# duylebkHCM/EyeDiseaseSegmentation

Hardware: NVIDIA B200
Metric: IDRiD-size (2848x4288) fundus images/s, 4 lesion models, sliding-window + 8-view D4 TTA + AUC-PR (higher is better)
Workload: dtype bf16

## Files before the change

eyediseasesegmentation_b200/csrc/conv3x3_wide_sm100.cu:

```cuda
#include "tc_ptx.cuh"
#include <algorithm>
#include <cstring>
#include <mutex>

namespace eds {

constexpr int kWideThreads = 320;
constexpr int kWideStagesMax = 4;
constexpr int kWideRows = 8, kWideSlabCols = 32, kWideOutCols = 30, kWideSlabRows = kWideRows + 2;

struct WideParams {
    CUtensorMap a_map;
    CUtensorMap a_map1;
    int k_split;
    CUtensorMap b_map;
    CUtensorMap y_map;
    const float* bias;
    const __nv_bfloat16* residual;
    __nv_bfloat16* y;
    int C, block_k, k_chunks, bn;
    int N, H, W, relu;
    int tiles_w, tiles_h, total_tiles;
    int stages, atom_bytes, a_slab_bytes, b_box_bytes, stage_bytes, tmem_cols;
    int b_resident, b_region_bytes;
    int staged, staging_off;
    uint32_t idesc, desc_hi;
};

__device__ __forceinline__ void wide_mbar_arrive(uint64_t* bar) {
    asm volatile("mbarrier.arrive.shared::cta.b64 _, [%0];" ::"r"(smem_u32(bar)) : "memory");
}

__global__ void __launch_bounds__(kWideThreads, 1)
conv3x3_wide_kernel(const __grid_constant__ WideParams p) {
    extern __shared__ uint8_t smem_raw[];
    uint8_t* smem = reinterpret_cast<uint8_t*>((reinterpret_cast<uintptr_t>(smem_raw) + 1023) & ~(uintptr_t)1023);
    uint8_t* ring = smem + p.b_region_bytes;
    uint64_t* full_bar = reinterpret_cast<uint64_t*>(ring + (size_t)p.stages * p.stage_bytes);
    uint64_t* empty_bar = full_bar + kWideStagesMax;
    uint64_t* tmem_full_bar = empty_bar + kWideStagesMax;
    uint64_t* tmem_empty_bar = tmem_full_bar + 2;
    uint64_t* b_bar = tmem_empty_bar + 2;
    uint32_t* tmem_slot = reinterpret_cast<uint32_t*>(b_bar + 1);
    float* s_bias = reinterpret_cast<float*>(full_bar + 16);
    if (threadIdx.x < (unsigned)p.bn) s_bias[threadIdx.x] = p.bias ? __ldg(p.bias + threadIdx.x) : 0.f;

    const int warp = threadIdx.x >> 5, lane = threadIdx.x & 31;
    if (warp == 0 && lane == 0) {
        prefetch_tmap(&p.a_map);
        prefetch_tmap(&p.a_map1);
        prefetch_tmap(&p.b_map);
        for (int s = 0; s < p.stages; ++s) {
            mbar_init(&full_bar[s], 1);
            mbar_init(&empty_bar[s], 1);
        }
        for (int m = 0; m < 2; ++m) {
            mbar_init(&tmem_full_bar[m], 1);
            mbar_init(&tmem_empty_bar[m], 4);
        }
        mbar_init(b_bar, 1);
        asm volatile("fence.mbarrier_init.release.cluster;" ::: "memory");
        asm volatile("fence.proxy.async.shared::cta;" ::: "memory");
    }
    if (warp == 1) tmem_alloc(tmem_slot, (uint32_t)p.tmem_cols);
    tc_fence_before();
    __syncthreads();
    tc_fence_after();
    const uint32_t tmem_base = *tmem_slot;
    const uint32_t n3 = 3u * (uint32_t)p.bn;

    if (warp == 0) {
        if (lane == 0) {
            int stage = 0;
            uint32_t phase = 0;
            const uint32_t a_tx = (uint32_t)(kWideSlabRows * 4 * p.atom_bytes), b_tx = (uint32_t)(9 * p.bn * p.block_k * 2);
            const uint32_t tx = p.b_resident ? a_tx : a_tx + b_tx;
            if (p.b_resident) {
                mbar_arrive_expect_tx(b_bar, b_tx * (uint32_t)p.k_chunks);
                for (int kc = 0; kc < p.k_chunks; ++kc)
                    for (int tap = 0; tap < 9; ++tap)
                        tma_load_2d(smem + (size_t)(kc * 9 + tap) * p.b_box_bytes, &p.b_map, b_bar,
                                    tap * p.C + kc * p.block_k, 0);
            }
            for (int tile = blockIdx.x; tile < p.total_tiles; tile += gridDim.x) {
                const int tw = tile % p.tiles_w;
                const int t2 = tile / p.tiles_w;
                const int th = t2 % p.tiles_h;
                const int n = t2 / p.tiles_h;
                const int w0 = tw * kWideOutCols, h0 = th * kWideRows;
                for (int kc = 0; kc < p.k_chunks; ++kc) {
                    mbar_wait(&empty_bar[stage], phase ^ 1u);
                    mbar_arrive_expect_tx(&full_bar[stage], tx);
                    uint8_t* sa = ring + (size_t)stage * p.stage_bytes;
                    uint8_t* sb = sa + p.a_slab_bytes;
                    if (kc < p.k_split)
                        tma_load_4d(sa, &p.a_map, &full_bar[stage], kc * p.block_k, w0 - 1, h0 - 1, n);
                    else
                        tma_load_4d(sa, &p.a_map1, &full_bar[stage], (kc - p.k_split) * p.block_k, w0 - 1, h0 - 1, n);
                    if (!p.b_resident)
                        for (int tap = 0; tap < 9; ++tap)
                            tma_load_2d(sb + tap * p.b_box_bytes, &p.b_map, &full_bar[stage], tap * p.C + kc * p.block_k, 0);
                    if (++stage == p.stages) { stage = 0; phase ^= 1u; }
                }
            }
        }
    } else if (warp == 1) {
        int stage = 0;
        uint32_t phase = 0;
        const uint32_t lo0 = desc_lo(smem_u32(ring)), blo0 = desc_lo(smem_u32(smem));
        const uint32_t stage16 = (uint32_t)p.stage_bytes >> 4, slab16 = (uint32_t)p.a_slab_bytes >> 4;
        const uint32_t bchunk16 = 9u * ((uint32_t)p.b_box_bytes >> 4);
        if (p.b_resident) mbar_wait(b_bar, 0);
        const uint32_t atom16 = (uint32_t)p.atom_bytes >> 4, brow16 = 3u * ((uint32_t)p.b_box_bytes >> 4);
        const uint32_t dhi_w = p.desc_hi, idesc = p.idesc;
        const int k_steps = p.block_k / 16;
        int t = 0;
        for (int tile = blockIdx.x; tile < p.total_tiles; tile += gridDim.x, ++t) {
            const uint32_t empty_parity = (uint32_t)((t & 1) ^ 1);
            for (int kc = 0; kc < p.k_chunks; ++kc) {
                mbar_wait(&full_bar[stage], phase);
                const uint32_t a_st = lo0 + (uint32_t)stage * stage16;
                const uint32_t b_st = p.b_resident ? blo0 + (uint32_t)kc * bchunk16 : a_st + slab16;
#pragma unroll
                for (int m = 0; m < 2; ++m) {
                    if (kc == 0) mbar_wait(&tmem_empty_bar[m], empty_parity);
                    tc_fence_after();
                    if (elect_one()) {
                        const uint32_t d = tmem_base + (uint32_t)m * n3;
#pragma unroll
                        for (int dhi = 0; dhi < 3; ++dhi) {
                            const uint32_t a_lo = a_st + (uint32_t)(m * 16 + dhi * 4) * atom16;
                            const uint32_t b_lo = b_st + (uint32_t)dhi * brow16;
                            for (int ks = 0; ks < k_steps; ++ks)
                                umma_bf16_lohi(d, a_lo + 2u * ks, b_lo + 2u * ks, dhi_w, idesc,
                                               (kc > 0 || dhi > 0 || ks > 0) ? 1u : 0u);
                        }
                    }
                    __syncwarp();
                    if (kc == p.k_chunks - 1) {
                        if (elect_one()) umma_commit(&tmem_full_bar[m]);
                        __syncwarp();
                    }
                }
                if (elect_one()) umma_commit(&empty_bar[stage]);
                __syncwarp();
                if (++stage == p.stages) { stage = 0; phase ^= 1u; }
            }
        }
    } else {
        const int q = warp & 3;
        const int m = (warp - 2) >> 2;
        const int bn = p.bn;
        uint8_t* stg = smem + p.staging_off + (size_t)(warp - 2) * 4096;
        const int pos = lane - 1;
        int t = 0;
        for (int tile = blockIdx.x; tile < p.total_tiles; tile += gridDim.x, ++t) {
            const int tw = tile % p.tiles_w;
            const int t2 = tile / p.tiles_w;
            const int th = t2 % p.tiles_h;
            const int n = t2 / p.tiles_h;
            const int ow = tw * kWideOutCols - 1 + lane;
            const bool col_ok = lane >= 1 && lane <= kWideOutCols && ow < p.W;
            {
                mbar_wait(&tmem_full_bar[m], (uint32_t)(t & 1));
                tc_fence_after();
                const int oh = th * kWideRows + m * 4 + q;
                const bool valid = col_ok && oh < p.H;
                const int64_t off = (((int64_t)n * p.H + oh) * p.W + ow) * bn;
                const uint32_t taddr = tmem_base + ((uint32_t)(q * 32) << 16) + (uint32_t)m * n3;
                if (p.staged) {
                    if (lane == 0) asm volatile("cp.async.bulk.wait_group.read 0;" ::: "memory");
                    __syncwarp();
                }
                for (int c = 0; c < bn; c += 16) {
                    uint32_t rl[16], rc[16], rr[16];
                    tmem_ld16_nowait(taddr + (uint32_t)c, rl);
                    tmem_ld16_nowait(taddr + (uint32_t)(bn + c), rc);
                    tmem_ld16_nowait(taddr + (uint32_t)(2 * bn + c), rr);
                    tmem_ld_wait();
                    float v[16];
#pragma unroll
                    for (int i = 0; i < 16; ++i) {
                        const float l = __shfl_up_sync(0xffffffffu, __uint_as_float(rl[i]), 1);
                        const float r = __shfl_down_sync(0xffffffffu, __uint_as_float(rr[i]), 1);
                        v[i] = (l + __uint_as_float(rc[i])) + r;
                    }
                    if (valid || (p.staged && pos >= 0 && pos < kWideOutCols)) {
                        {
                            const float4* b4 = reinterpret_cast<const float4*>(s_bias + c);
#pragma unroll
                            for (int i = 0; i < 4; ++i) {
                                const float4 b = b4[i];
                                v[4 * i] += b.x; v[4 * i + 1] += b.y; v[4 * i + 2] += b.z; v[4 * i + 3] += b.w;
                            }
                        }
                        if (p.residual && valid) {
                            float r0[8], r1[8];
                            Vec8<__nv_bfloat16>::ld(p.residual + off + c, r0);
                            Vec8<__nv_bfloat16>::ld(p.residual + off + c + 8, r1);
#pragma unroll
                            for (int i = 0; i < 8; ++i) { v[i] += r0[i]; v[8 + i] += r1[i]; }
                        }
                        if (p.relu) {
#pragma unroll
                            for (int i = 0; i < 16; ++i) v[i] = fmaxf(v[i], 0.f);
                        }
                        float o0[8], o1[8];
#pragma unroll
                        for (int i = 0; i < 8; ++i) { o0[i] = v[i]; o1[i] = v[8 + i]; }
                        if (p.staged) {
                            const uint32_t j = (uint32_t)c >> 3, sw = (uint32_t)pos & 7u;
                            Vec8<__nv_bfloat16>::st(reinterpret_cast<__nv_bfloat16*>(stg + pos * 128 + ((j ^ sw) << 4)), o0);
                            Vec8<__nv_bfloat16>::st(reinterpret_cast<__nv_bfloat16*>(stg + pos * 128 + (((j + 1) ^ sw) << 4)), o1);
                        } else {
                            Vec8<__nv_bfloat16>::st(p.y + off + c, o0);
                            Vec8<__nv_bfloat16>::st(p.y + off + c + 8, o1);
                        }
                    }
                }
                if (p.staged) {
                    asm volatile("fence.proxy.async.shared::cta;" ::: "memory");
                    __syncwarp();
                    if (lane == 0 && oh < p.H) {
                        asm volatile(
                            "cp.async.bulk.tensor.4d.global.shared::cta.bulk_group [%0, {%2, %3, %4, %5}], [%1];"
                            ::"l"(&p.y_map), "r"(smem_u32(stg)), "r"(0), "r"(tw * kWideOutCols), "r"(oh), "r"(n)
                            : "memory");
                        asm volatile("cp.async.bulk.commit_group;" ::: "memory");
                    }
                }
                tc_fence_before();
                __syncwarp();
                if (lane == 0) wide_mbar_arrive(&tmem_empty_bar[m]);
            }
        }
        if (p.staged && lane == 0) asm volatile("cp.async.bulk.wait_group 0;" ::: "memory");
    }

    tc_fence_before();
    __syncthreads();
    if (warp == 1) tmem_dealloc(tmem_base, (uint32_t)p.tmem_cols);
}

static PerDevice g_wide_once;
static int g_wide_sms = 148;

static int wide_init() {
    return g_wide_once.run([](int dev) {
        cudaError_t e = cudaFuncSetAttribute(conv3x3_wide_kernel, cudaFuncAttributeMaxDynamicSharedMemorySize, 227 * 1024);
        if (e != cudaSuccess) {
            set_error("conv3x3_wide: cannot opt in to 227 KB shared memory: %s", cudaGetErrorString(e));
            return (int)EDS_ERR_CUDA;
        }
        int sms = 0;
        if (cudaDeviceGetAttribute(&sms, cudaDevAttrMultiProcessorCount, dev) == cudaSuccess && sms > 0) g_wide_sms = sms;
        return (int)EDS_OK;
    });
}

}

using namespace eds;

extern "C" int eds_conv3x3_wide_supported(int C, int Cout, int R, int S, int stride, int pad) {
    return R == 3 && S == 3 && stride == 1 && pad == 1 && C >= 16 && C % 16 == 0 && Cout >= 16 && Cout % 16 == 0 &&
           Cout <= 64;
}

static int wide_launch(const void* x, int C0, const void* x1, int C1, int N, int H, int W, const void* w,
                       const float* bias, int Cout, int relu, const void* residual, void* y, void* stream) {
    const int C = C0 + C1;
    EDS_REQUIRE(x && w && y, "conv3x3_wide: null pointer");
    EDS_REQUIRE(C0 >= 16 && C0 % 16 == 0 && C1 >= 0 && C1 % 16 == 0 && (x1 != nullptr) == (C1 > 0),
                "conv3x3_wide: C0=%d C1=%d must be multiples of 16", C0, C1);
    EDS_REQUIRE(N > 0 && H > 0 && W > 0, "conv3x3_wide: bad shape N=%d H=%d W=%d", N, H, W);
    EDS_REQUIRE(eds_conv3x3_wide_supported(C, Cout, 3, 3, 1, 1),
                "conv3x3_wide: C=%d Cout=%d outside the supported range (multiples of 16, Cout <= 64)", C, Cout);
    EDS_REQUIRE((((uintptr_t)x | (uintptr_t)x1 | (uintptr_t)w | (uintptr_t)y | (uintptr_t)residual | (uintptr_t)bias) &
                 15) == 0, "conv3x3_wide: pointers must be 16-byte aligned");
    if (int rc = igemm_init()) return rc;
    if (int rc = wide_init()) return rc;

    WideParams p;
    memset(&p, 0, sizeof(p));
    p.bias = bias;
    p.residual = (const __nv_bfloat16*)residual;
    p.y = (__nv_bfloat16*)y;
    p.C = C;
    p.block_k = ((C0 | C1) % 64 == 0) ? 64 : ((C0 | C1) % 32 == 0 ? 32 : 16);
    p.k_chunks = C / p.block_k;
    p.k_split = C0 / p.block_k;
    p.bn = Cout;
    p.N = N; p.H = H; p.W = W; p.relu = relu;
    p.tiles_w = ceil_div(W, kWideOutCols);
    p.tiles_h = ceil_div(H, kWideRows);
    const int64_t total = (int64_t)p.tiles_w * p.tiles_h * N;
    EDS_REQUIRE(total < (1ll << 31), "conv3x3_wide: too many tiles");
    p.total_tiles = (int)total;

    const CUtensorMapSwizzle swz = p.block_k == 64 ? CU_TENSOR_MAP_SWIZZLE_128B
                                  : p.block_k == 32 ? CU_TENSOR_MAP_SWIZZLE_64B : CU_TENSOR_MAP_SWIZZLE_32B;
    const uint32_t layout = p.block_k == 64 ? 2u : (p.block_k == 32 ? 4u : 6u);
    p.atom_bytes = 8 * p.block_k * 2;
    const uint32_t sbo = (uint32_t)p.atom_bytes >> 4;
    p.desc_hi = sbo | (1u << 14) | (layout << 29);
    p.idesc = (1u << 4) | (1u << 7) | (1u << 10) | ((uint32_t)((3 * p.bn) >> 3) << 17) | ((uint32_t)(128 >> 4) << 24);
    p.a_slab_bytes = (kWideSlabRows * 4 * p.atom_bytes + 1023) & ~1023;
    p.b_box_bytes = p.bn * p.block_k * 2;
    const int barrier_bytes = 128 + 64 * 4;
    const int budget = 227 * 1024 - 1024 - barrier_bytes;
    const int b_all = p.k_chunks * 9 * p.b_box_bytes;
    p.b_resident = b_all + 3 * p.a_slab_bytes <= budget;
    p.b_region_bytes = p.b_resident ? ((b_all + 1023) & ~1023) : 0;
    p.stage_bytes = p.b_resident ? p.a_slab_bytes : ((p.a_slab_bytes + 9 * p.b_box_bytes + 1023) & ~1023);
    p.stages = std::min(kWideStagesMax, (budget - p.b_region_bytes) / p.stage_bytes);
    EDS_REQUIRE(p.stages >= 2, "conv3x3_wide: a stage of %d B leaves no room for double buffering", p.stage_bytes);
    int cols = 32;
    while (cols < 6 * p.bn) cols <<= 1;
    p.tmem_cols = cols;
    const int after_bars = p.b_region_bytes + p.stages * p.stage_bytes + barrier_bytes;
    p.staging_off = (after_bars + 1023) & ~1023;
    p.staged = p.bn == 64 && p.block_k == 64 && p.staging_off + 8 * 4096 + 1024 <= 227 * 1024;
    const size_t smem = (p.staged ? (size_t)p.staging_off + 8 * 4096 : (size_t)after_bars) + 1024;
    EDS_REQUIRE(smem <= 227 * 1024 && p.tmem_cols <= 512, "conv3x3_wide: tile does not fit (smem %zu, tmem %d)", smem,
                p.tmem_cols);

    {
        cuuint64_t dims[4] = {(cuuint64_t)C0, (cuuint64_t)W, (cuuint64_t)H, (cuuint64_t)N};
        cuuint64_t strides[3] = {(cuuint64_t)C0 * 2, (cuuint64_t)W * C0 * 2, (cuuint64_t)H * W * C0 * 2};
        cuuint32_t box[4] = {(cuuint32_t)p.block_k, (cuuint32_t)kWideSlabCols, (cuuint32_t)kWideSlabRows, 1u};
        if (int rc = tmap_encode_bf16(&p.a_map, x, 4, dims, strides, box, swz, "wide input")) return rc;
        p.a_map1 = p.a_map;
    }
    if (x1) {
        cuuint64_t dims[4] = {(cuuint64_t)C1, (cuuint64_t)W, (cuuint64_t)H, (cuuint64_t)N};
        cuuint64_t strides[3] = {(cuuint64_t)C1 * 2, (cuuint64_t)W * C1 * 2, (cuuint64_t)H * W * C1 * 2};
        cuuint32_t box[4] = {(cuuint32_t)p.block_k, (cuuint32_t)kWideSlabCols, (cuuint32_t)kWideSlabRows, 1u};
        if (int rc = tmap_encode_bf16(&p.a_map1, x1, 4, dims, strides, box, swz, "wide second input")) return rc;
    }
    {
        cuuint64_t dims[2] = {(cuuint64_t)9 * C, (cuuint64_t)Cout};
        cuuint64_t strides[1] = {(cuuint64_t)9 * C * 2};
        cuuint32_t box[2] = {(cuuint32_t)p.block_k, (cuuint32_t)p.bn};
        if (int rc = tmap_encode_bf16(&p.b_map, w, 2, dims, strides, box, swz, "wide weights")) return rc;
    }
    if (p.staged) {
        cuuint64_t dims[4] = {(cuuint64_t)Cout, (cuuint64_t)W, (cuuint64_t)H, (cuuint64_t)N};
        cuuint64_t strides[3] = {(cuuint64_t)Cout * 2, (cuuint64_t)W * Cout * 2, (cuuint64_t)H * W * Cout * 2};
        cuuint32_t box[4] = {64u, (cuuint32_t)kWideOutCols, 1u, 1u};
        if (int rc = tmap_encode_bf16(&p.y_map, y, 4, dims, strides, box, CU_TENSOR_MAP_SWIZZLE_128B, "wide output")) return rc;
    }
    const int grid = (int)std::min<int64_t>(total, g_wide_sms);
    conv3x3_wide_kernel<<<grid, kWideThreads, smem, as_stream(stream)>>>(p);
    return check_launch("conv3x3_wide_kernel");
}

extern "C" int eds_conv3x3_wide_bf16(const void* x, int N, int H, int W, int C, const void* w, const float* bias,
                                     int Cout, int relu, const void* residual, void* y, void* stream) {
    return wide_launch(x, C, nullptr, 0, N, H, W, w, bias, Cout, relu, residual, y, stream);
}

extern "C" int eds_conv3x3_wide_bf16_2src(const void* x0, int C0, const void* x1, int C1, int N, int H, int W,
                                          const void* w, const float* bias, int Cout, int relu, const void* residual,
                                          void* y, void* stream) {
    EDS_REQUIRE(x1 && C1 > 0, "conv3x3_wide_2src: second input missing");
    return wide_launch(x0, C0, x1, C1, N, H, W, w, bias, Cout, relu, residual, y, stream);
}
```

eyediseasesegmentation_b200/csrc/tc_ptx.cuh:

```cuda
#pragma once
#include "common.cuh"
#include <cuda.h>

namespace eds {

__device__ __forceinline__ uint32_t smem_u32(const void* p) { return (uint32_t)__cvta_generic_to_shared(p); }

__device__ __forceinline__ void mbar_init(uint64_t* bar, uint32_t count) {
    asm volatile("mbarrier.init.shared::cta.b64 [%0], %1;" ::"r"(smem_u32(bar)), "r"(count) : "memory");
}
__device__ __forceinline__ void mbar_arrive_expect_tx(uint64_t* bar, uint32_t bytes) {
    asm volatile("mbarrier.arrive.expect_tx.shared::cta.b64 _, [%0], %1;" ::"r"(smem_u32(bar)), "r"(bytes)
                 : "memory");
}
__device__ __forceinline__ bool mbar_try_wait(uint64_t* bar, uint32_t parity) {
    uint32_t ok;
    asm volatile(
        "{\n\t.reg .pred p;\n\t"
        "mbarrier.try_wait.parity.shared::cta.b64 p, [%1], %2;\n\t"
        "selp.u32 %0, 1, 0, p;\n\t}"
        : "=r"(ok)
        : "r"(smem_u32(bar)), "r"(parity)
        : "memory");
    return ok != 0;
}
__device__ __forceinline__ void mbar_wait(uint64_t* bar, uint32_t parity) {
    if (mbar_try_wait(bar, parity)) return;
    const long long t0 = clock64();
    while (!mbar_try_wait(bar, parity)) {
        if (clock64() - t0 > 4000000000LL) {
            printf("eds conv_igemm: mbarrier timeout (block %d thread %d)\n", (int)blockIdx.x, (int)threadIdx.x);
            __trap();
        }
    }
}
__device__ __forceinline__ void tma_load_4d(void* dst, const CUtensorMap* map, uint64_t* bar, int c0, int c1, int c2,
                                            int c3) {
    asm volatile(
        "cp.async.bulk.tensor.4d.shared::cluster.global.mbarrier::complete_tx::bytes [%0], [%1, {%3, %4, %5, %6}], [%2];"
        ::"r"(smem_u32(dst)), "l"(map), "r"(smem_u32(bar)), "r"(c0), "r"(c1), "r"(c2), "r"(c3)
        : "memory");
}
__device__ __forceinline__ void tma_load_2d(void* dst, const CUtensorMap* map, uint64_t* bar, int c0, int c1) {
    asm volatile(
        "cp.async.bulk.tensor.2d.shared::cluster.global.mbarrier::complete_tx::bytes [%0], [%1, {%3, %4}], [%2];"
        ::"r"(smem_u32(dst)), "l"(map), "r"(smem_u32(bar)), "r"(c0), "r"(c1)
        : "memory");
}
__device__ __forceinline__ void prefetch_tmap(const CUtensorMap* map) {
    asm volatile("prefetch.tensormap [%0];" ::"l"(map) : "memory");
}
__device__ __forceinline__ void tc_fence_before() { asm volatile("tcgen05.fence::before_thread_sync;" ::: "memory"); }
__device__ __forceinline__ void tc_fence_after() { asm volatile("tcgen05.fence::after_thread_sync;" ::: "memory"); }
__device__ __forceinline__ void tmem_alloc(uint32_t* dst, uint32_t cols) {
    asm volatile("tcgen05.alloc.cta_group::1.sync.aligned.shared::cta.b32 [%0], %1;" ::"r"(smem_u32(dst)), "r"(cols)
                 : "memory");
    asm volatile("tcgen05.relinquish_alloc_permit.cta_group::1.sync.aligned;" ::: "memory");
}
__device__ __forceinline__ void tmem_dealloc(uint32_t addr, uint32_t cols) {
    asm volatile("tcgen05.dealloc.cta_group::1.sync.aligned.b32 %0, %1;" ::"r"(addr), "r"(cols) : "memory");
}
__device__ __forceinline__ void umma_bf16(uint32_t tmem_d, uint64_t desc_a, uint64_t desc_b, uint32_t idesc,
                                          uint32_t accumulate) {
    asm volatile(
        "{\n\t.reg .pred p;\n\t"
        "setp.ne.b32 p, %4, 0;\n\t"
        "tcgen05.mma.cta_group::1.kind::f16 [%0], %1, %2, %3, p;\n\t}"
        ::"r"(tmem_d), "l"(desc_a), "l"(desc_b), "r"(idesc), "r"(accumulate)
        : "memory");
}
__device__ __forceinline__ void umma_commit(uint64_t* bar) {
    asm volatile("tcgen05.commit.cta_group::1.mbarrier::arrive::one.shared::cluster.b64 [%0];" ::"r"(smem_u32(bar))
                 : "memory");
}
__device__ __forceinline__ void tmem_ld16(uint32_t taddr, uint32_t (&r)[16]) {
    asm volatile(
        "tcgen05.ld.sync.aligned.32x32b.x16.b32 "
        "{%0, %1, %2, %3, %4, %5, %6, %7, %8, %9, %10, %11, %12, %13, %14, %15}, [%16];"
        : "=r"(r[0]), "=r"(r[1]), "=r"(r[2]), "=r"(r[3]), "=r"(r[4]), "=r"(r[5]), "=r"(r[6]), "=r"(r[7]), "=r"(r[8]),
          "=r"(r[9]), "=r"(r[10]), "=r"(r[11]), "=r"(r[12]), "=r"(r[13]), "=r"(r[14]), "=r"(r[15])
        : "r"(taddr)
        : "memory");
    asm volatile("tcgen05.wait::ld.sync.aligned;" ::: "memory");
}

__device__ __forceinline__ void tmem_ld16_nowait(uint32_t taddr, uint32_t (&r)[16]) {
    asm volatile(
        "tcgen05.ld.sync.aligned.32x32b.x16.b32 "
        "{%0, %1, %2, %3, %4, %5, %6, %7, %8, %9, %10, %11, %12, %13, %14, %15}, [%16];"
        : "=r"(r[0]), "=r"(r[1]), "=r"(r[2]), "=r"(r[3]), "=r"(r[4]), "=r"(r[5]), "=r"(r[6]), "=r"(r[7]), "=r"(r[8]),
          "=r"(r[9]), "=r"(r[10]), "=r"(r[11]), "=r"(r[12]), "=r"(r[13]), "=r"(r[14]), "=r"(r[15])
        : "r"(taddr)
        : "memory");
}
__device__ __forceinline__ void tmem_ld_wait() { asm volatile("tcgen05.wait::ld.sync.aligned;" ::: "memory"); }

__device__ __forceinline__ bool elect_one() {
    uint32_t pred;
    asm volatile(
        "{\n\t.reg .pred p;\n\t"
        "elect.sync _|p, 0xffffffff;\n\t"
        "selp.u32 %0, 1, 0, p;\n\t}"
        : "=r"(pred));
    return pred != 0;
}
__device__ __forceinline__ void umma_bf16_lohi(uint32_t tmem_d, uint32_t a_lo, uint32_t b_lo, uint32_t desc_hi,
                                               uint32_t idesc, uint32_t accumulate) {
    asm volatile(
        "{\n\t.reg .pred p;\n\t.reg .b64 da, db;\n\t"
        "setp.ne.b32 p, %5, 0;\n\t"
        "mov.b64 da, {%1, %3};\n\t"
        "mov.b64 db, {%2, %3};\n\t"
        "tcgen05.mma.cta_group::1.kind::f16 [%0], da, db, %4, p;\n\t}"
        ::"r"(tmem_d), "r"(a_lo), "r"(b_lo), "r"(desc_hi), "r"(idesc), "r"(accumulate)
        : "memory");
}
__device__ __forceinline__ uint32_t desc_lo(uint32_t saddr) { return ((saddr & 0x3FFFFu) >> 4) | (1u << 16); }

__device__ __forceinline__ uint64_t make_desc(uint32_t saddr, uint32_t desc_hi) {
    return (uint64_t)(((saddr & 0x3FFFFu) >> 4) | (1u << 16)) | ((uint64_t)desc_hi << 32);
}


int tmap_encode_bf16(CUtensorMap* map, const void* base, int rank, const cuuint64_t* dims, const cuuint64_t* strides,
                     const cuuint32_t* box, CUtensorMapSwizzle swz, const char* what);
int igemm_init();

}
```

Before: 1.890.

## Run wide 3x3 conv as 2-CTA cluster pairs with split weight loads

Adds a cta_group::2 variant of the wide implicit-GEMM 3x3 convolution. Two CTAs in a cluster each load their own activation slab and half of the weight boxes, and the leader issues M=256 paired UMMAs, with commits multicast to both CTAs and cross-CTA TMEM-empty arrivals. This halves per-CTA weight shared-memory traffic and footprint, allowing more pipeline stages (max raised to 5). It adds cluster synchronisation, a drain loop and an occupancy query, and risks load imbalance from odd tile counts and extra handshake latency.

```diff
diff --git a/eyediseasesegmentation_b200/csrc/conv3x3_wide_sm100.cu b/eyediseasesegmentation_b200/csrc/conv3x3_wide_sm100.cu
--- a/eyediseasesegmentation_b200/csrc/conv3x3_wide_sm100.cu
+++ b/eyediseasesegmentation_b200/csrc/conv3x3_wide_sm100.cu
@@ -2,11 +2,13 @@
 #include <algorithm>
 #include <cstring>
 #include <mutex>
+#include <utility>
+#include <vector>
 
 namespace eds {
 
 constexpr int kWideThreads = 320;
-constexpr int kWideStagesMax = 4;
+constexpr int kWideStagesMax = 5;
 constexpr int kWideRows = 8, kWideSlabCols = 32, kWideOutCols = 30, kWideSlabRows = kWideRows + 2;
 
 struct WideParams {
@@ -20,17 +22,30 @@
     __nv_bfloat16* y;
     int C, block_k, k_chunks, bn;
     int N, H, W, relu;
-    int tiles_w, tiles_h, total_tiles;
+    int tiles_w, tiles_h, total_tiles, total_pairs;
     int stages, atom_bytes, a_slab_bytes, b_box_bytes, stage_bytes, tmem_cols;
     int b_resident, b_region_bytes;
     int staged, staging_off;
     uint32_t idesc, desc_hi;
 };
 
-__device__ __forceinline__ void wide_mbar_arrive(uint64_t* bar) {
-    asm volatile("mbarrier.arrive.shared::cta.b64 _, [%0];" ::"r"(smem_u32(bar)) : "memory");
-}
-
+template <int kCtas> __device__ __forceinline__ void wide_commit(uint64_t* bar) {
+    if constexpr (kCtas == 2) umma_commit_pair(bar);
+    else umma_commit(bar);
+}
+template <int kCtas>
+__device__ __forceinline__ void wide_tma_4d(void* dst, const CUtensorMap* map, uint64_t* bar, int c0, int c1, int c2,
+                                            int c3) {
+    if constexpr (kCtas == 2) tma_load_4d_pair(dst, map, cluster_addr(bar, 0), c0, c1, c2, c3);
+    else tma_load_4d(dst, map, bar, c0, c1, c2, c3);
+}
+template <int kCtas>
+__device__ __forceinline__ void wide_tma_2d(void* dst, const CUtensorMap* map, uint64_t* bar, int c0, int c1) {
+    if constexpr (kCtas == 2) tma_load_2d_pair(dst, map, cluster_addr(bar, 0), c0, c1);
+    else tma_load_2d(dst, map, bar, c0, c1);
+}
+
+template <int kCtas>
 __global__ void __launch_bounds__(kWideThreads, 1)
 conv3x3_wide_kernel(const __grid_constant__ WideParams p) {
     extern __shared__ uint8_t smem_raw[];
@@ -46,6 +61,8 @@
     if (threadIdx.x < (unsigned)p.bn) s_bias[threadIdx.x] = p.bias ? __ldg(p.bias + threadIdx.x) : 0.f;
 
     const int warp = threadIdx.x >> 5, lane = threadIdx.x & 31;
+    const uint32_t rank = kCtas == 2 ? cluster_ctarank() : 0u;
+    const int pair0 = (int)blockIdx.x / kCtas, pair_step = (int)gridDim.x / kCtas;
     if (warp == 0 && lane == 0) {
         prefetch_tmap(&p.a_map);
         prefetch_tmap(&p.a_map1);
@@ -56,15 +73,19 @@
         }
         for (int m = 0; m < 2; ++m) {
             mbar_init(&tmem_full_bar[m], 1);
-            mbar_init(&tmem_empty_bar[m], 4);
+            mbar_init(&tmem_empty_bar[m], 4 * kCtas);
         }
         mbar_init(b_bar, 1);
         asm volatile("fence.mbarrier_init.release.cluster;" ::: "memory");
         asm volatile("fence.proxy.async.shared::cta;" ::: "memory");
     }
-    if (warp == 1) tmem_alloc(tmem_slot, (uint32_t)p.tmem_cols);
+    if (warp == 1) {
+        if constexpr (kCtas == 2) tmem_alloc_pair(tmem_slot, (uint32_t)p.tmem_cols);
+        else tmem_alloc(tmem_slot, (uint32_t)p.tmem_cols);
+    }
     tc_fence_before();
-    __syncthreads();
+    if constexpr (kCtas == 2) cluster_sync();
+    else __syncthreads();
     tc_fence_after();
     const uint32_t tmem_base = *tmem_slot;
     const uint32_t n3 = 3u * (uint32_t)p.bn;
@@ -73,16 +94,23 @@
         if (lane == 0) {
             int stage = 0;
             uint32_t phase = 0;
-            const uint32_t a_tx = (uint32_t)(kWideSlabRows * 4 * p.atom_bytes), b_tx = (uint32_t)(9 * p.bn * p.block_k * 2);
-            const uint32_t tx = p.b_resident ? a_tx : a_tx + b_tx;
+            const int hb = p.bn >> 1, nb = 6 / kCtas;
+            const uint32_t a_tx = (uint32_t)(kWideSlabRows * 4 * p.atom_bytes), b_tx = (uint32_t)(3 * nb * p.b_box_bytes);
+            const uint32_t tx = (uint32_t)kCtas * (p.b_resident ? a_tx : a_tx + b_tx);
+            auto load_b = [&](uint8_t* sb, uint64_t* bar, int kc) {
+                for (int dh = 0; dh < 3; ++dh)
+                    for (int i = 0; i < nb; ++i) {
+                        const int j = nb * (int)rank + i;
+                        wide_tma_2d<kCtas>(sb + (dh * nb + i) * p.b_box_bytes, &p.b_map, bar,
+                                           (dh * 3 + (j >> 1)) * p.C + kc * p.block_k, (j & 1) * hb);
+                    }
+            };
             if (p.b_resident) {
-                mbar_arrive_expect_tx(b_bar, b_tx * (uint32_t)p.k_chunks);
-                for (int kc = 0; kc < p.k_chunks; ++kc)
-                    for (int tap = 0; tap < 9; ++tap)
-                        tma_load_2d(smem + (size_t)(kc * 9 + tap) * p.b_box_bytes, &p.b_map, b_bar,
-                                    tap * p.C + kc * p.block_k, 0);
+                if (rank == 0) mbar_arrive_expect_tx(b_bar, (uint32_t)kCtas * b_tx * (uint32_t)p.k_chunks);
+                for (int kc = 0; kc < p.k_chunks; ++kc) load_b(smem + (size_t)kc * b_tx, b_bar, kc);
             }
-            for (int tile = blockIdx.x; tile < p.total_tiles; tile += gridDim.x) {
+            for (int pt = pair0; pt < p.total_pairs; pt += pair_step) {
+                const int tile = kCtas * pt + (int)rank;
                 const int tw = tile % p.tiles_w;
                 const int t2 = tile / p.tiles_w;
                 const int th = t2 % p.tiles_h;
@@ -90,77 +118,92 @@
                 const int w0 = tw * kWideOutCols, h0 = th * kWideRows;
                 for (int kc = 0; kc < p.k_chunks; ++kc) {
                     mbar_wait(&empty_bar[stage], phase ^ 1u);
-                    mbar_arrive_expect_tx(&full_bar[stage], tx);
+                    if (rank == 0) mbar_arrive_expect_tx(&full_bar[stage], tx);
+                    uint64_t* bar = &full_bar[stage];
                     uint8_t* sa = ring + (size_t)stage * p.stage_bytes;
                     uint8_t* sb = sa + p.a_slab_bytes;
                     if (kc < p.k_split)
-                        tma_load_4d(sa, &p.a_map, &full_bar[stage], kc * p.block_k, w0 - 1, h0 - 1, n);
+                        wide_tma_4d<kCtas>(sa, &p.a_map, bar, kc * p.block_k, w0 - 1, h0 - 1, n);
                     else
-                        tma_load_4d(sa, &p.a_map1, &full_bar[stage], (kc - p.k_split) * p.block_k, w0 - 1, h0 - 1, n);
-                    if (!p.b_resident)
-                        for (int tap = 0; tap < 9; ++tap)
-                            tma_load_2d(sb + tap * p.b_box_bytes, &p.b_map, &full_bar[stage], tap * p.C + kc * p.block_k, 0);
+                        wide_tma_4d<kCtas>(sa, &p.a_map1, bar, (kc - p.k_split) * p.block_k, w0 - 1, h0 - 1, n);
+                    if (!p.b_resident) load_b(sb, bar, kc);
                     if (++stage == p.stages) { stage = 0; phase ^= 1u; }
                 }
             }
+            for (int s = 0; s < p.stages; ++s) {
+                mbar_wait(&empty_bar[stage], phase ^ 1u);
+                if (++stage == p.stages) { stage = 0; phase ^= 1u; }
+            }
         }
     } else if (warp == 1) {
-        int stage = 0;
-        uint32_t phase = 0;
-        const uint32_t lo0 = desc_lo(smem_u32(ring)), blo0 = desc_lo(smem_u32(smem));
-        const uint32_t stage16 = (uint32_t)p.stage_bytes >> 4, slab16 = (uint32_t)p.a_slab_bytes >> 4;
-        const uint32_t bchunk16 = 9u * ((uint32_t)p.b_box_bytes >> 4);
-        if (p.b_resident) mbar_wait(b_bar, 0);
-        const uint32_t atom16 = (uint32_t)p.atom_bytes >> 4, brow16 = 3u * ((uint32_t)p.b_box_bytes >> 4);
-        const uint32_t dhi_w = p.desc_hi, idesc = p.idesc;
-        const int k_steps = p.block_k / 16;
-        int t = 0;
-        for (int tile = blockIdx.x; tile < p.total_tiles; tile += gridDim.x, ++t) {
-            const uint32_t empty_parity = (uint32_t)((t & 1) ^ 1);
-            for (int kc = 0; kc < p.k_chunks; ++kc) {
-                mbar_wait(&full_bar[stage], phase);
-                const uint32_t a_st = lo0 + (uint32_t)stage * stage16;
-                const uint32_t b_st = p.b_resident ? blo0 + (uint32_t)kc * bchunk16 : a_st + slab16;
-#pragma unroll
-                for (int m = 0; m < 2; ++m) {
-                    if (kc == 0) mbar_wait(&tmem_empty_bar[m], empty_parity);
-                    tc_fence_after();
-                    if (elect_one()) {
-                        const uint32_t d = tmem_base + (uint32_t)m * n3;
-#pragma unroll
-                        for (int dhi = 0; dhi < 3; ++dhi) {
-                            const uint32_t a_lo = a_st + (uint32_t)(m * 16 + dhi * 4) * atom16;
-                            const uint32_t b_lo = b_st + (uint32_t)dhi * brow16;
-                            for (int ks = 0; ks < k_steps; ++ks)
-                                umma_bf16_lohi(d, a_lo + 2u * ks, b_lo + 2u * ks, dhi_w, idesc,
-                                               (kc > 0 || dhi > 0 || ks > 0) ? 1u : 0u);
+        if (rank == 0) {
+            int stage = 0;
+            uint32_t phase = 0;
+            const uint32_t lo0 = desc_lo(smem_u32(ring)), blo0 = desc_lo(smem_u32(smem));
+            const uint32_t stage16 = (uint32_t)p.stage_bytes >> 4, slab16 = (uint32_t)p.a_slab_bytes >> 4;
+            const uint32_t brow16 = (uint32_t)(6 / kCtas) * ((uint32_t)p.b_box_bytes >> 4), bchunk16 = 3u * brow16;
+            if (p.b_resident) mbar_wait(b_bar, 0);
+            const uint32_t atom16 = (uint32_t)p.atom_bytes >> 4;
+            const uint32_t dhi_w = p.desc_hi, idesc = p.idesc;
+            const int k_steps = p.block_k / 16;
+            int t = 0;
+            for (int pt = pair0; pt < p.total_pairs; pt += pair_step, ++t) {
+                const uint32_t empty_parity = (uint32_t)((t & 1) ^ 1);
+                for (int kc = 0; kc < p.k_chunks; ++kc) {
+                    mbar_wait(&full_bar[stage], phase);
+                    const uint32_t a_st = lo0 + (uint32_t)stage * stage16;
+                    const uint32_t b_st = p.b_resident ? blo0 + (uint32_t)kc * bchunk16 : a_st + slab16;
+#pragma unroll
+                    for (int m = 0; m < 2; ++m) {
+                        if (kc == 0) {
+                            if constexpr (kCtas == 2) mbar_wait_cluster(&tmem_empty_bar[m], empty_parity);
+                            else mbar_wait(&tmem_empty_bar[m], empty_parity);
+                        }
+                        tc_fence_after();
+                        if (elect_one()) {
+                            const uint32_t d = tmem_base + (uint32_t)m * n3;
+#pragma unroll
+                            for (int dhi = 0; dhi < 3; ++dhi) {
+                                const uint32_t a_lo = a_st + (uint32_t)(m * 16 + dhi * 4) * atom16;
+                                const uint32_t b_lo = b_st + (uint32_t)dhi * brow16;
+                                for (int ks = 0; ks < k_steps; ++ks) {
+                                    const uint32_t acc = (kc > 0 || dhi > 0 || ks > 0) ? 1u : 0u;
+                                    if constexpr (kCtas == 2)
+                                        umma_bf16_pair_lohi(d, a_lo + 2u * ks, b_lo + 2u * ks, dhi_w, idesc, acc);
+                                    else
+                                        umma_bf16_lohi(d, a_lo + 2u * ks, b_lo + 2u * ks, dhi_w, idesc, acc);
+                                }
+                            }
+                        }
+                        __syncwarp();
+                        if (kc == p.k_chunks - 1) {
+                            if (elect_one()) wide_commit<kCtas>(&tmem_full_bar[m]);
+                            __syncwarp();
                         }
                     }
+                    if (elect_one()) wide_commit<kCtas>(&empty_bar[stage]);
                     __syncwarp();
-                    if (kc == p.k_chunks - 1) {
-                        if (elect_one()) umma_commit(&tmem_full_bar[m]);
-                        __syncwarp();
-                    }
-                }
-                if (elect_one()) umma_commit(&empty_bar[stage]);
-                __syncwarp();
-                if (++stage == p.stages) { stage = 0; phase ^= 1u; }
+                    if (++stage == p.stages) { stage = 0; phase ^= 1u; }
+                }
             }
         }
     } else {
         const int q = warp & 3;
         const int m = (warp - 2) >> 2;
         const int bn = p.bn;
+        const uint32_t empty_bar_leader = kCtas == 2 ? cluster_addr(&tmem_empty_bar[m], 0) : 0u;
         uint8_t* stg = smem + p.staging_off + (size_t)(warp - 2) * 4096;
         const int pos = lane - 1;
         int t = 0;
-        for (int tile = blockIdx.x; tile < p.total_tiles; tile += gridDim.x, ++t) {
+        for (int pt = pair0; pt < p.total_pairs; pt += pair_step, ++t) {
+            const int tile = kCtas * pt + (int)rank;
+            const bool tile_ok = tile < p.total_tiles;
             const int tw = tile % p.tiles_w;
             const int t2 = tile / p.tiles_w;
             const int th = t2 % p.tiles_h;
             const int n = t2 / p.tiles_h;
             const int ow = tw * kWideOutCols - 1 + lane;
-            const bool col_ok = lane >= 1 && lane <= kWideOutCols && ow < p.W;
+            const bool col_ok = tile_ok && lane >= 1 && lane <= kWideOutCols && ow < p.W;
             {
                 mbar_wait(&tmem_full_bar[m], (uint32_t)(t & 1));
                 tc_fence_after();
@@ -221,7 +264,7 @@
                 if (p.staged) {
                     asm volatile("fence.proxy.async.shared::cta;" ::: "memory");
                     __syncwarp();
-                    if (lane == 0 && oh < p.H) {
+                    if (lane == 0 && tile_ok && oh < p.H) {
                         asm volatile(
                             "cp.async.bulk.tensor.4d.global.shared::cta.bulk_group [%0, {%2, %3, %4, %5}], [%1];"
                             ::"l"(&p.y_map), "r"(smem_u32(stg)), "r"(0), "r"(tw * kWideOutCols), "r"(oh), "r"(n)
@@ -231,29 +274,78 @@
                 }
                 tc_fence_before();
                 __syncwarp();
-                if (lane == 0) wide_mbar_arrive(&tmem_empty_bar[m]);
+                if (lane == 0) {
+                    if constexpr (kCtas == 2) mbar_arrive_cluster(empty_bar_leader);
+                    else asm volatile("mbarrier.arrive.shared::cta.b64 _, [%0];" ::"r"(smem_u32(&tmem_empty_bar[m])) : "memory");
+                }
             }
         }
         if (p.staged && lane == 0) asm volatile("cp.async.bulk.wait_group 0;" ::: "memory");
     }
 
     tc_fence_before();
-    __syncthreads();
-    if (warp == 1) tmem_dealloc(tmem_base, (uint32_t)p.tmem_cols);
+    if constexpr (kCtas == 2) cluster_sync();
+    else __syncthreads();
+    tc_fence_after();
+    if (warp == 1) {
+        if constexpr (kCtas == 2) tmem_dealloc_pair(tmem_base, (uint32_t)p.tmem_cols);
+        else tmem_dealloc(tmem_base, (uint32_t)p.tmem_cols);
+    }
 }
 
 static PerDevice g_wide_once;
-static int g_wide_sms = 148;
+static int g_wide_sms[kMaxDevices];
+
+static cudaLaunchConfig_t wide_pair_config(int grid, size_t smem, cudaStream_t stream, cudaLaunchAttribute* attr) {
+    cudaLaunchConfig_t cfg = {};
+    cfg.gridDim = dim3((unsigned)grid);
+    cfg.blockDim = dim3(kWideThreads);
+    cfg.dynamicSmemBytes = smem;
+    cfg.stream = stream;
+    attr->id = cudaLaunchAttributeClusterDimension;
+    attr->val.clusterDim.x = 2;
+    attr->val.clusterDim.y = 1;
+    attr->val.clusterDim.z = 1;
+    cfg.attrs = attr;
+    cfg.numAttrs = 1;
+    return cfg;
+}
+
+static int wide_max_pairs(size_t smem) {
+    static std::mutex mu;
+    static std::vector<std::pair<std::pair<int, size_t>, int>> cache;
+    int dev = 0;
+    if (cudaGetDevice(&dev) != cudaSuccess) return 0;
+    std::lock_guard<std::mutex> lock(mu);
+    for (const auto& e : cache)
+        if (e.first.first == dev && e.first.second == smem) return e.second;
+    cudaLaunchAttribute attr;
+    const cudaLaunchConfig_t cfg = wide_pair_config(2 * g_wide_sms[dev], smem, nullptr, &attr);
+    int pairs = 0;
+    if (cudaOccupancyMaxActiveClusters(&pairs, conv3x3_wide_kernel<2>, &cfg) != cudaSuccess || pairs <= 0) {
+        (void)cudaGetLastError();
+        return 0;
+    }
+    cache.push_back({{dev, smem}, pairs});
+    return pairs;
+}
 
 static int wide_init() {
     return g_wide_once.run([](int dev) {
-        cudaError_t e = cudaFuncSetAttribute(conv3x3_wide_kernel, cudaFuncAttributeMaxDynamicSharedMemorySize, 227 * 1024);
+        cudaError_t e = cudaFuncSetAttribute(conv3x3_wide_kernel<1>, cudaFuncAttributeMaxDynamicSharedMemorySize, 227 * 1024);
+        if (e == cudaSuccess)
+            e = cudaFuncSetAttribute(conv3x3_wide_kernel<2>, cudaFuncAttributeMaxDynamicSharedMemorySize, 227 * 1024);
         if (e != cudaSuccess) {
             set_error("conv3x3_wide: cannot opt in to 227 KB shared memory: %s", cudaGetErrorString(e));
             return (int)EDS_ERR_CUDA;
         }
         int sms = 0;
-        if (cudaDeviceGetAttribute(&sms, cudaDevAttrMultiProcessorCount, dev) == cudaSuccess && sms > 0) g_wide_sms = sms;
+        e = cudaDeviceGetAttribute(&sms, cudaDevAttrMultiProcessorCount, dev);
+        if (e != cudaSuccess || sms < 2) {
+            set_error("conv3x3_wide: cannot read the SM count: %s", cudaGetErrorString(e));
+            return (int)EDS_ERR_CUDA;
+        }
+        g_wide_sms[dev] = sms;
         return (int)EDS_OK;
     });
 }
@@ -288,8 +380,6 @@
     p.y = (__nv_bfloat16*)y;
     p.C = C;
     p.block_k = ((C0 | C1) % 64 == 0) ? 64 : ((C0 | C1) % 32 == 0 ? 32 : 16);
-    p.k_chunks = C / p.block_k;
-    p.k_split = C0 / p.block_k;
     p.bn = Cout;
     p.N = N; p.H = H; p.W = W; p.relu = relu;
     p.tiles_w = ceil_div(W, kWideOutCols);
@@ -298,29 +388,44 @@
     EDS_REQUIRE(total < (1ll << 31), "conv3x3_wide: too many tiles");
     p.total_tiles = (int)total;
 
+    const int barrier_bytes = 128 + 64 * 4;
+    const int budget = 227 * 1024 - 1024 - barrier_bytes;
+    int ctas = 0;
+    for (;;) {
+        p.k_chunks = C / p.block_k;
+        p.k_split = C0 / p.block_k;
+        p.atom_bytes = 8 * p.block_k * 2;
+        p.a_slab_bytes = (kWideSlabRows * 4 * p.atom_bytes + 1023) & ~1023;
+        p.b_box_bytes = (p.bn / 2) * p.block_k * 2;
+        const int b_whole = p.k_chunks * 18 * p.b_box_bytes;
+        if (ctas == 0) ctas = b_whole + 3 * p.a_slab_bytes <= budget ? 1 : 2;
+        const int b_all = b_whole / ctas;
+        p.b_resident = b_all + 3 * p.a_slab_bytes <= budget;
+        p.b_region_bytes = p.b_resident ? ((b_all + 1023) & ~1023) : 0;
+        p.stage_bytes = p.b_resident ? p.a_slab_bytes : ((p.a_slab_bytes + 18 / ctas * p.b_box_bytes + 1023) & ~1023);
+        const int staging_bytes = 8 * 4096;
+        const int ring_room = budget - p.b_region_bytes;
+        p.staged = p.bn == 64 && ring_room - staging_bytes - 1024 >= 2 * p.stage_bytes;
+        p.stages = std::min(kWideStagesMax, (ring_room - (p.staged ? staging_bytes + 1024 : 0)) / p.stage_bytes);
+        if (ctas == 2 && !p.b_resident && p.block_k == 64 && p.stages < 3) {
+            p.block_k = 32;
+            continue;
+        }
+        break;
+    }
+    EDS_REQUIRE(p.stages >= 2, "conv3x3_wide: a stage of %d B leaves no room for double buffering", p.stage_bytes);
+    p.total_pairs = (int)ceil_div64(total, ctas);
     const CUtensorMapSwizzle swz = p.block_k == 64 ? CU_TENSOR_MAP_SWIZZLE_128B
                                   : p.block_k == 32 ? CU_TENSOR_MAP_SWIZZLE_64B : CU_TENSOR_MAP_SWIZZLE_32B;
     const uint32_t layout = p.block_k == 64 ? 2u : (p.block_k == 32 ? 4u : 6u);
-    p.atom_bytes = 8 * p.block_k * 2;
-    const uint32_t sbo = (uint32_t)p.atom_bytes >> 4;
-    p.desc_hi = sbo | (1u << 14) | (layout << 29);
-    p.idesc = (1u << 4) | (1u << 7) | (1u << 10) | ((uint32_t)((3 * p.bn) >> 3) << 17) | ((uint32_t)(128 >> 4) << 24);
-    p.a_slab_bytes = (kWideSlabRows * 4 * p.atom_bytes + 1023) & ~1023;
-    p.b_box_bytes = p.bn * p.block_k * 2;
-    const int barrier_bytes = 128 + 64 * 4;
-    const int budget = 227 * 1024 - 1024 - barrier_bytes;
-    const int b_all = p.k_chunks * 9 * p.b_box_bytes;
-    p.b_resident = b_all + 3 * p.a_slab_bytes <= budget;
-    p.b_region_bytes = p.b_resident ? ((b_all + 1023) & ~1023) : 0;
-    p.stage_bytes = p.b_resident ? p.a_slab_bytes : ((p.a_slab_bytes + 9 * p.b_box_bytes + 1023) & ~1023);
-    p.stages = std::min(kWideStagesMax, (budget - p.b_region_bytes) / p.stage_bytes);
-    EDS_REQUIRE(p.stages >= 2, "conv3x3_wide: a stage of %d B leaves no room for double buffering", p.stage_bytes);
+    p.desc_hi = ((uint32_t)p.atom_bytes >> 4) | (1u << 14) | (layout << 29);
+    p.idesc = (1u << 4) | (1u << 7) | (1u << 10) | ((uint32_t)((3 * p.bn) >> 3) << 17) |
+              ((uint32_t)(128 * ctas >> 4) << 24);
     int cols = 32;
     while (cols < 6 * p.bn) cols <<= 1;
     p.tmem_cols = cols;
     const int after_bars = p.b_region_bytes + p.stages * p.stage_bytes + barrier_bytes;
     p.staging_off = (after_bars + 1023) & ~1023;
-    p.staged = p.bn == 64 && p.block_k == 64 && p.staging_off + 8 * 4096 + 1024 <= 227 * 1024;
     const size_t smem = (p.staged ? (size_t)p.staging_off + 8 * 4096 : (size_t)after_bars) + 1024;
     EDS_REQUIRE(smem <= 227 * 1024 && p.tmem_cols <= 512, "conv3x3_wide: tile does not fit (smem %zu, tmem %d)", smem,
                 p.tmem_cols);
@@ -341,7 +446,7 @@
     {
         cuuint64_t dims[2] = {(cuuint64_t)9 * C, (cuuint64_t)Cout};
         cuuint64_t strides[1] = {(cuuint64_t)9 * C * 2};
-        cuuint32_t box[2] = {(cuuint32_t)p.block_k, (cuuint32_t)p.bn};
+        cuuint32_t box[2] = {(cuuint32_t)p.block_k, (cuuint32_t)(p.bn / 2)};
         if (int rc = tmap_encode_bf16(&p.b_map, w, 2, dims, strides, box, swz, "wide weights")) return rc;
     }
     if (p.staged) {
@@ -350,8 +455,23 @@
         cuuint32_t box[4] = {64u, (cuuint32_t)kWideOutCols, 1u, 1u};
         if (int rc = tmap_encode_bf16(&p.y_map, y, 4, dims, strides, box, CU_TENSOR_MAP_SWIZZLE_128B, "wide output")) return rc;
     }
-    const int grid = (int)std::min<int64_t>(total, g_wide_sms);
-    conv3x3_wide_kernel<<<grid, kWideThreads, smem, as_stream(stream)>>>(p);
+    int dev = 0;
+    EDS_REQUIRE(cudaGetDevice(&dev) == cudaSuccess, "conv3x3_wide: no current device");
+    if (ctas == 1) {
+        const int grid = std::min(p.total_pairs, g_wide_sms[dev]);
+        conv3x3_wide_kernel<1><<<grid, kWideThreads, smem, as_stream(stream)>>>(p);
+        return check_launch("conv3x3_wide_kernel");
+    }
+    const int max_pairs = wide_max_pairs(smem);
+    EDS_REQUIRE(max_pairs > 0, "conv3x3_wide: a CTA pair with %zu B of shared memory cannot be resident", smem);
+    const int pairs = std::min({p.total_pairs, max_pairs, g_wide_sms[dev] / 2});
+    cudaLaunchAttribute attr;
+    const cudaLaunchConfig_t cfg = wide_pair_config(2 * pairs, smem, as_stream(stream), &attr);
+    const cudaError_t e = cudaLaunchKernelEx(&cfg, conv3x3_wide_kernel<2>, p);
+    if (e != cudaSuccess) {
+        set_error("conv3x3_wide: launch of the CTA-pair kernel failed: %s", cudaGetErrorString(e));
+        return (int)EDS_ERR_CUDA;
+    }
     return check_launch("conv3x3_wide_kernel");
 }
 
diff --git a/eyediseasesegmentation_b200/csrc/tc_ptx.cuh b/eyediseasesegmentation_b200/csrc/tc_ptx.cuh
--- a/eyediseasesegmentation_b200/csrc/tc_ptx.cuh
+++ b/eyediseasesegmentation_b200/csrc/tc_ptx.cuh
@@ -117,6 +117,85 @@
 }
 __device__ __forceinline__ uint32_t desc_lo(uint32_t saddr) { return ((saddr & 0x3FFFFu) >> 4) | (1u << 16); }
 
+__device__ __forceinline__ uint32_t cluster_ctarank() {
+    uint32_t r;
+    asm volatile("mov.u32 %0, %%cluster_ctarank;" : "=r"(r));
+    return r;
+}
+__device__ __forceinline__ void cluster_sync() {
+    asm volatile("barrier.cluster.arrive.release.aligned;\n\tbarrier.cluster.wait.acquire.aligned;" ::: "memory");
+}
+__device__ __forceinline__ uint32_t cluster_addr(const void* p, uint32_t rank) {
+    uint32_t r;
+    asm volatile("mapa.shared::cluster.u32 %0, %1, %2;" : "=r"(r) : "r"(smem_u32(p)), "r"(rank));
+    return r;
+}
+__device__ __forceinline__ bool mbar_try_wait_cluster(uint64_t* bar, uint32_t parity) {
+    uint32_t ok;
+    asm volatile(
+        "{\n\t.reg .pred p;\n\t"
+        "mbarrier.try_wait.parity.acquire.cluster.shared::cta.b64 p, [%1], %2;\n\t"
+        "selp.u32 %0, 1, 0, p;\n\t}"
+        : "=r"(ok)
+        : "r"(smem_u32(bar)), "r"(parity)
+        : "memory");
+    return ok != 0;
+}
+__device__ __forceinline__ void mbar_wait_cluster(uint64_t* bar, uint32_t parity) {
+    if (mbar_try_wait_cluster(bar, parity)) return;
+    const long long t0 = clock64();
+    while (!mbar_try_wait_cluster(bar, parity)) {
+        if (clock64() - t0 > 4000000000LL) {
+            printf("eds conv_igemm: mbarrier timeout (block %d thread %d)\n", (int)blockIdx.x, (int)threadIdx.x);
+            __trap();
+        }
+    }
+}
+__device__ __forceinline__ void mbar_arrive_cluster(uint32_t cluster_bar) {
+    asm volatile("mbarrier.arrive.release.cluster.shared::cluster.b64 _, [%0];" ::"r"(cluster_bar) : "memory");
+}
+__device__ __forceinline__ void tma_load_4d_pair(void* dst, const CUtensorMap* map, uint32_t cluster_bar, int c0,
+                                                 int c1, int c2, int c3) {
+    asm volatile(
+        "cp.async.bulk.tensor.4d.cta_group::2.shared::cluster.global.mbarrier::complete_tx::bytes"
+        " [%0], [%1, {%3, %4, %5, %6}], [%2];"
+        ::"r"(smem_u32(dst)), "l"(map), "r"(cluster_bar), "r"(c0), "r"(c1), "r"(c2), "r"(c3)
+        : "memory");
+}
+__device__ __forceinline__ void tma_load_2d_pair(void* dst, const CUtensorMap* map, uint32_t cluster_bar, int c0,
+                                                 int c1) {
+    asm volatile(
+        "cp.async.bulk.tensor.2d.cta_group::2.shared::cluster.global.mbarrier::complete_tx::bytes"
+        " [%0], [%1, {%3, %4}], [%2];"
+        ::"r"(smem_u32(dst)), "l"(map), "r"(cluster_bar), "r"(c0), "r"(c1)
+        : "memory");
+}
+__device__ __forceinline__ void tmem_alloc_pair(uint32_t* dst, uint32_t cols) {
+    asm volatile("tcgen05.alloc.cta_group::2.sync.aligned.shared::cta.b32 [%0], %1;" ::"r"(smem_u32(dst)), "r"(cols)
+                 : "memory");
+    asm volatile("tcgen05.relinquish_alloc_permit.cta_group::2.sync.aligned;" ::: "memory");
+}
+__device__ __forceinline__ void tmem_dealloc_pair(uint32_t addr, uint32_t cols) {
+    asm volatile("tcgen05.dealloc.cta_group::2.sync.aligned.b32 %0, %1;" ::"r"(addr), "r"(cols) : "memory");
+}
+__device__ __forceinline__ void umma_bf16_pair_lohi(uint32_t tmem_d, uint32_t a_lo, uint32_t b_lo, uint32_t desc_hi,
+                                                    uint32_t idesc, uint32_t accumulate) {
+    asm volatile(
+        "{\n\t.reg .pred p;\n\t.reg .b64 da, db;\n\t"
+        "setp.ne.b32 p, %5, 0;\n\t"
+        "mov.b64 da, {%1, %3};\n\t"
+        "mov.b64 db, {%2, %3};\n\t"
+        "tcgen05.mma.cta_group::2.kind::f16 [%0], da, db, %4, p;\n\t}"
+        ::"r"(tmem_d), "r"(a_lo), "r"(b_lo), "r"(desc_hi), "r"(idesc), "r"(accumulate)
+        : "memory");
+}
+__device__ __forceinline__ void umma_commit_pair(uint64_t* bar) {
+    asm volatile(
+        "tcgen05.commit.cta_group::2.mbarrier::arrive::one.shared::cluster.multicast::cluster.b64 [%0], %1;"
+        ::"r"(smem_u32(bar)), "h"((uint16_t)3)
+        : "memory");
+}
+
 __device__ __forceinline__ uint64_t make_desc(uint32_t saddr, uint32_t desc_hi) {
     return (uint64_t)(((saddr & 0x3FFFFu) >> 4) | (1u << 16)) | ((uint64_t)desc_hi << 32);
 }
```

After: 1.853, median of 6. 0.98x the previous value.
